# gillesdegottex/percivaltts

Hardware: AMD Instinct MI355X
Metric: acoustic frames/sec per WGAN-GP critic+gen step (higher is better)
Workload: dtype f32

## Files before the change

include/percival_hip.h:

```cpp
#ifndef PERCIVAL_HIP_H
#define PERCIVAL_HIP_H

#include <stddef.h>
#include <stdint.h>

#ifdef __cplusplus
extern "C" {
#endif

#define PTTS_OK            0
#define PTTS_EINVAL       -1
#define PTTS_ELAUNCH      -2
#define PTTS_EWORKSPACE   -3
#define PTTS_EDEVICE      -4

#define PTTS_IN_NONE     0
#define PTTS_IN_LRELU    1
#define PTTS_IN_MASKMUL  2

#define PTTS_PAD_SAME    0
#define PTTS_PAD_CAUSAL  1

#define PTTS_ACT_NONE    0
#define PTTS_ACT_LRELU   1
#define PTTS_ACT_SIGMOID 2
#define PTTS_ACT_TANH    3

const char* ptts_version(void);
const char* ptts_device_arch(void);
const char* ptts_last_error(void);
int ptts_device_status(unsigned* word_out);
int ptts_device_status_clear(void);
unsigned* ptts_device_status_word(void);
int ptts_device_status_message(unsigned word, char* buf, size_t n);
int ptts_set_deterministic(int on);
int ptts_get_deterministic(void);
int ptts_set_bf16_products(int on);
int ptts_get_bf16_products(void);

int ptts_conv2d_fwd(const float* x, const float* w, const float* bias ,
                    const float* in_scale , const float* in_shift ,
                    const float* mask_src ,
                    float* y,
                    int B, int T, int F, int Cin, int Cout, int KT, int KF,
                    int dil_t, int pad_mode, int in_mode, float alpha, void* stream);

size_t ptts_conv2d_bwd_workspace_bytes(int B, int T, int F, int Cin, int Cout, int KT, int KF, int dil_t);
int ptts_conv2d_bwd(const float* dy, const float* x, const float* w,
                    const float* in_scale, const float* in_shift, const float* mask_src,
                    float* dx, float* dw, float* dbias, float* dscale, float* dshift,
                    void* workspace, size_t workspace_bytes,
                    int B, int T, int F, int Cin, int Cout, int KT, int KF,
                    int dil_t, int pad_mode, int in_mode, float alpha, void* stream);

int ptts_conv2d_bwd_partials(const float* dy, const float* x, const float* w, const float* mask_src,
                             float* dx, void* workspace, size_t workspace_bytes, int* nblocks_out,
                             int B, int T, int F, int Cin, int Cout, int KT, int KF,
                             int dil_t, int pad_mode, int in_mode, float alpha, void* stream);
typedef struct ptts_conv2d_reduce_desc {
    const float* partials;
    int nblocks, npart, nw, cout;
    float* dw; float* dbias;
} ptts_conv2d_reduce_desc;
int ptts_conv2d_reduce_grouped(const ptts_conv2d_reduce_desc* descs, int n, void* stream);

int ptts_conv2d_mfma_supported(int F, int Cin, int Cout, int KT, int KF, int dil_t);
size_t ptts_conv2d_mfma_table_bytes(int KT);
int ptts_conv2d_mfma_tables(const float* w, void* table_fwd, void* table_bwd, int KT, int KF, int Cin, int Cout,
                            int planes , void* stream);
int ptts_conv2d_mfma_tables_grouped(const float* const* w, void* const* table_fwd, void* const* table_bwd, int n, int planes,
                                    void* stream);
int ptts_conv2d_mfma_fwd(const void* x, const void* table, const float* bias, const float* in_scale, const float* in_shift,
                         const void* mask_src, const void* out_mask, void* y,
                         int B, int T, int F, int KT, int dil_t, int pad_t, int in_mode, float alpha,
                         int planes, int in_bf16, int out_bf16, void* stream);
int ptts_conv2d_mfma_fwd_stats_supported(int F, int dil_t, int in_mode);
int ptts_conv2d_mfma_fwd_stats(const float* x, const void* table, const float* bias, const float* in_scale, const float* in_shift,
                               float* y, int B, int T, int F, int KT, int pad_t, int in_mode, float alpha,
                               double* stats, int capacity_rows, int* nrows_out, void* stream);
size_t ptts_conv2d_mfma_wgrad_workspace_bytes(int B, int T);
int ptts_conv2d_mfma_wgrad_partials(const void* dy, const void* x, const void* mask_src, void* workspace,
                                    size_t workspace_bytes, int* nblocks_out, int* npart_out, int B, int T, int F,
                                    int KT, int dil_t, int pad_t, int in_mode, float alpha,
                                    int planes, int x_bf16, int dy_bf16, void* stream);
size_t ptts_conv2d_mfma_bwd_fused_workspace_bytes(int B, int T);
int ptts_conv2d_mfma_bwd_fused_supported(int F, int dil_t, int planes);
int ptts_conv2d_mfma_bwd_fused(const void* p, const void* q, const void* mask_src, const void* table, void* y,
                               void* workspace, size_t workspace_bytes, int* nblocks_out, int* npart_out,
                               int B, int T, int F, int KT, int pad_t, int kind, float alpha, void* stream);
int ptts_conv2d_mfma_bwd_fused_affine(const float* p, const float* q, const void* table, float* y, void* workspace, size_t workspace_bytes,
                                      int* nblocks_out, int* npart_out, int B, int T, int F, int KT, int pad_t, float alpha,
                                      const float* q_scale, const float* q_shift, void* stream);
int ptts_conv2d_mfma_debug(int flags, void* stamp_buf);

int ptts_conv2d_chain_supported(int F, int L, int Cin0, int C, int KT, int KF);
int ptts_conv2d_chain_debug(void* stamp_buf);
size_t ptts_conv2d_chain_tables_bytes(void);
size_t ptts_conv2d_chain_partials_bytes(int L);
long long ptts_conv2d_chain_map_elems(int B, int T, int F);
int ptts_conv2d_chain_tables(const float* const* w, const float* const* b, void* tables, int L, int cin0, void* stream);
int ptts_conv2d_chain_fwd(const float* x0, long long ldx, const void* tables, void* maps, void* a_last,
                          int B, int T, int F, int L, float alpha, void* stream);
int ptts_conv2d_chain_bwd(const void* d_last, int d_bf16, const float* x0, long long ldx, const void* maps, const void* a_last,
                          const void* tables, float* partials, size_t partials_bytes, int* nblocks_out, int* npart_out,
                          int B, int T, int F, int L, int cin0, float alpha, void* stream);
int ptts_conv2d_chain_bwd_data(const void* d_last, int d_bf16, const void* maps, const void* a_last, const void* tables,
                               void* gmaps, float* g0, int B, int T, int F, int L, float alpha, void* stream);
int ptts_conv2d_chain_second(const float* u0, const void* gmaps, const void* maps, const void* a_last, const void* tables,
                             void* out, int out_bf16, float* partials, size_t partials_bytes, int* nblocks_out, int* npart_out,
                             int B, int T, int F, int L, int cin0, float alpha, void* stream);

int ptts_gemm(const float* A, const float* Bm, const float* bias, float* C,
              int M, int N, int K,
              int transA, long long lda, long long rows_per_seg, long long seg_stride,
              int transB, long long ldb, long long ldc,
              int in_mode, const float* in_scale, const float* in_shift, const float* mask_src,
              float alpha, int accumulate, const float* out_mask, float* colsum_b, void* stream);

typedef struct ptts_wgrad_desc {
    const float* A; const float* B; float* C; float* colsum_b;
    const float* in_scale; const float* in_shift; const float* mask_src;
    int M, N, K;
    long long lda, ldb, ldc;
    int in_mode; float alpha;
} ptts_wgrad_desc;
int ptts_gemm_wgrad_grouped(const ptts_wgrad_desc* descs, int n, void* stream);

size_t ptts_dense_planes_bytes(int N, int K);
int ptts_split3_dense_weight(const float* w, long long ldw, int K, int N, int transposed, void* planes, void* stream);
typedef struct ptts_dense_split_desc {
    const float* w; void* planes;
    long long ldw;
    int K, N, transposed, reserved;
} ptts_dense_split_desc;
int ptts_split3_dense_weight_grouped(const ptts_dense_split_desc* descs, int n, void* stream);
int ptts_split3_frame_windows(const float* x, int B, int T, int C, int NS, int S, int row_off, int P, int kvalid,
                              void* planes, long long stride_planes_bytes, void* stream);
int ptts_split3_dense_weight_strided(const float* w, long long stride_w, void* planes, long long stride_planes_bytes, int n,
                                     long long ldw, int K, int N, int transposed, void* stream);
int ptts_dense_bf16x6_supported(int M, int N, int K, long long lda, long long ldc);
typedef struct ptts_dense_wgrad_reduce_desc {
    const float* partials;
    int split, Kin, N;
    long long ldc;
    float* C; float* colsum_b;
} ptts_dense_wgrad_reduce_desc;
int ptts_dense_wgrad_bf16x6_supported(int Kin, int N, int M, long long lda, long long ldb);
size_t ptts_dense_wgrad_workspace_bytes(int Kin, int N, int M);
int ptts_dense_wgrad_bf16x6_partials(const float* A, const float* dY, const float* mask_src, const float* in_scale,
                                     const float* in_shift, void* workspace, size_t workspace_bytes, int* split_out,
                                     int Kin, int N, int M, long long lda, long long ldb, int in_mode, float alpha,
                                     void* stream);
int ptts_dense_wgrad_reduce_grouped(const ptts_dense_wgrad_reduce_desc* descs, int n, void* stream);
int ptts_dense_wgrad_bf16x6(const float* A, const float* dY, const float* mask_src, const float* in_scale,
                            const float* in_shift, float* C, float* colsum_b, void* workspace, size_t workspace_bytes,
                            int Kin, int N, int M, long long lda, long long ldb, long long ldc, int in_mode, float alpha,
                            void* stream);
int ptts_dense_bf16x6(const float* A, const void* planes, const float* bias, float* C, int M, int N, int K,
                      long long lda, long long ldc, int in_mode, const float* in_scale, const float* in_shift,
                      const float* mask_src, float alpha, int accumulate, const float* out_mask, void* stream);
int ptts_dense_bf16x6_res(const float* A, const void* planes, const float* bias, float* C, int M, int N, int K,
                          long long lda, long long ldc, int in_mode, const float* in_scale, const float* in_shift,
                          const float* mask_src, float alpha, const float* res, int res_rows, long long ldr,
                          const float* out_mask, void* stream);
int ptts_dense_bf16x6_stats_rows(int M, int N);
int ptts_dense_bf16x6_stats(const float* A, const void* planes, const float* bias, float* C, int M, int N, int K,
                            long long lda, long long ldc, int in_mode, const float* in_scale, const float* in_shift,
                            float alpha, double* stats, int capacity_rows, int* nrows_out, void* stream);
int ptts_dense_bf16x6_bwd_affine(const float* A, const void* planes, float* C, int M, int N, int K, long long lda, long long ldc,
                                 const float* z, const float* scale, const float* shift, float alpha,
                                 double* stats, int capacity_rows, int* nrows_out, void* stream);
int ptts_partial_rows_sum(const double* partials, int nrows, int ncols, double* out, void* stream);
int ptts_dft_mirror(float* Ap, int NB, int B, int Cin, int Kh, void* stream);

int ptts_conv1d_freq_kernel_planes(const float* w, const float* tw, void* planes, int NB, int KW, int Cin, int N, int Kh, void* stream);

int ptts_transpose_batched(const float* src, float* dst, int nb, int rows, int cols, void* stream);
int ptts_conv1d_freq_wgrad_combine(const float* out2, float* dW, int KW, int Cin, int N, int Kh, void* stream);

size_t ptts_conv1d_freq_wgrad_inverse_workspace_bytes(int KW, int Cin, int N);
int ptts_conv1d_freq_wgrad_inverse(const float* Gt, const float* t2, float* dW, void* workspace, size_t workspace_bytes,
                                   int NB, int NBp, int KW, int Cin, int N, int Kh, void* stream);

#define PTTS_PLANES_ROWS 0x100
typedef struct ptts_dense_rows_desc {
    const float* B;
    long long strideB, ldb;
    int windows, nB, T, NS, S, row_off;
    int kvalid, mirror_cols;
} ptts_dense_rows_desc;
int ptts_dense_bf16x6_batched(const float* A, long long strideA, const void* planes, long long stride_planes_bytes,
                              const float* bias, float* C, long long strideC, int nbatch, int M, int N, int K,
                              long long lda, long long ldc, int planes_count, void* stream);
int ptts_set_dense_batched_resident(int on);
int ptts_dense_batched_resident_enabled(void);
int ptts_dense_batched_resident_eligible(long long strideA, int M, int N, int K, int planes_count);
int ptts_dense_tn_bf16x6_batched(const float* A, long long strideA, const float* B, long long strideB, float* C, long long strideC,
                                 int nbatch, int M, int Kin, int N, long long lda, long long ldb, long long ldc, int planes_count,
                                 void* stream);

int ptts_split3_frames(const float* x, void* p1, void* p2, void* p3, int B, int T, int C, int pad_left, int pad_right,
                       int Cp, void* stream);
int ptts_split3_weight_t(const float* w, void* p1, void* p2, void* p3, int KW, int C, int N, int Cp, void* stream);
int ptts_conv1d_bf16x6(const void* a1, const void* a2, const void* a3, const void* bt1, const void* bt2, const void* bt3,
                       const float* bias, float* y, int B, int T, int KW, int Cp, int N, void* stream);

int ptts_split3_frames_t(const float* x, void* p1, void* p2, void* p3, int B, int T, int C, int pad_left, int Tp, int Crows,
                         long long Pp, void* stream);
int ptts_conv1d_wgrad_bf16x6(const void* xt1, const void* xt2, const void* xt3, const void* yt1, const void* yt2,
                             const void* yt3, float* dw, int B, int T, int KW, int C, int N, int Crows, long long Pp,
                             void* stream);

int ptts_transpose_frames(const float* x, float* out, int B, int T, int C, int pad_left, int Tp, int Crows, long long Pp,
                          void* stream);
int ptts_conv1d_wgrad_t(const float* xt, const float* yt, float* dw, float* db, int B, int T, int KW, int C, int N, int Crows,
                        long long Pp, void* stream);

size_t ptts_colstats_workspace_bytes(long long rows, int C);
int ptts_colstats(const float* x, long long rows, int C,
                  int in_mode, const float* in_scale, const float* in_shift, const float* mask_src, float alpha,
                  double* sums , void* workspace, size_t workspace_bytes, void* stream);

int ptts_bn_finalize(const double* sums, long long count, const float* gamma, const float* beta,
                     float* moving_mean, float* moving_var, float eps, float momentum,
                     int training, int update_moving, int unbiased_moving, int C,
                     float* scale, float* shift, float* mean , float* rstd , void* stream);

int ptts_bn_batch_stats_supported(long long rows, int C);
int ptts_bn_batch_stats(const float* x, long long rows, int C, const float* gamma, const float* beta,
                        float* moving_mean, float* moving_var, float eps, float momentum, int update_moving, int unbiased_moving,
                        float* scale, float* shift, float* mean , float* rstd ,
                        void* workspace, size_t workspace_bytes, int* counter, void* stream);

int ptts_bn_finalize_partials(const double* partials, int nrows, long long rows, int C, const float* gamma, const float* beta,
                              float* moving_mean, float* moving_var, float eps, float momentum, int update_moving, int unbiased_moving,
                              float* scale, float* shift, float* mean , float* rstd , void* stream);

int ptts_bn_bwd_coefs(const float* dscale, const float* dshift, const float* mean, const float* rstd,
                      const float* gamma , long long count, int C,
                      float* dgamma, float* dbeta, float* c0, float* c2, void* stream);
int ptts_bn_bwd_coefs_acc(const float* dscale, const float* dshift, const float* mean, const float* rstd,
                      const float* gamma , long long count, int C,
                      float* dgamma, float* dbeta, float* c0, float* c2, void* stream);

int ptts_affine_act(const float* x, const float* scale, const float* shift, float* y,
                    long long rows, int C, int act, float alpha, void* stream);
int ptts_affine_act_bwd(const float* dy, const float* x, const float* y, const float* scale, const float* shift,
                        float* dx, double* dsums ,
                        void* workspace, size_t workspace_bytes,
                        long long rows, int C, int act, float alpha, void* stream);
int ptts_gated_mul_fwd(const float* a, const float* b, float* y, long long n, void* stream);
int ptts_gated_mul_bwd(const float* dy, const float* a, const float* b, float* da, float* db, long long n, void* stream);

int ptts_axpby_cols(const float* a, const float* c1, const float* x, const float* c2, const float* c0,
                    float* out, long long rows, int C, void* stream);

int ptts_gp_interpolate(const float* real, const float* fake, const float* alpha_b , float* out,
                        int B, long long TD, void* stream);
int ptts_gp_sqnorm(const float* g, float* out, int B, long long TD, void* stream);
int ptts_gp_penalty(const float* sq , float* penalty , float* coef , int B, void* stream);
int ptts_gp_scale_rows(const float* g, const float* coef, const float* upstream , float* dg,
                       int B, long long TD, void* stream);

int ptts_mean_scaled(const float* v, long long n, float sign, float* out, void* stream);
int ptts_wlse_fwd(const float* y, const float* yhat, const float* w , float* out,
                  long long rows, int D, void* stream);
int ptts_wlse_bwd(const float* y, const float* yhat, const float* w, const float* upstream, float* dyhat,
                  long long rows, int D, void* stream);

int ptts_weight_clip(float* p, long long n, float lo, float hi, void* stream);

int ptts_adam_keras_step(float* p, const float* g, float* m, float* v, long long n,
                         float lr, float b1, float b2, float eps, float gscale,
                         int* step , void* stream);

size_t ptts_lstm_fwd_workspace_bytes(int B, int T, int H, int ndir);
int ptts_lstm_fwd(const float* xproj, const float* U, float* h_out, float* gates, float* c_out,
                  void* workspace, size_t workspace_bytes,
                  int B, int T, int H, int ndir, int reverse, void* stream);
size_t ptts_lstm_bwd_workspace_bytes(int B, int T, int H, int ndir);
int ptts_lstm_bwd(const float* dh_out , const float* U, const float* gates, const float* c_out,
                  float* dgates, void* workspace, size_t workspace_bytes,
                  int B, int T, int H, int ndir, int reverse, void* stream);
int ptts_lstm_graph_stats(unsigned long long* hits, unsigned long long* captures, unsigned long long* direct);

size_t ptts_gru_fwd_workspace_bytes(int B, int T, int H, int ndir);
int ptts_gru_fwd(const float* xproj, const float* U, float* h_out, float* gates, float* rh,
                 void* workspace, size_t workspace_bytes, int B, int T, int H, int ndir, void* stream);
size_t ptts_gru_bwd_workspace_bytes(int B, int T, int H, int ndir);
int ptts_gru_bwd(const float* dh_out , const float* U, const float* h_out, const float* gates,
                 float* dgates, void* workspace, size_t workspace_bytes, int B, int T, int H, int ndir, void* stream);

size_t ptts_mlpg_workspace_bytes(int B, int T, int D);
int ptts_mlpg(const float* y, const float* mean, const float* std, const float* var, int var_per_frame,
              const float* wins, const int* lengths, float* out, void* workspace, size_t workspace_bytes,
              int B, int T, int D, int K, void* stream);

#define PTTS_NORM_MEANSTD 0
#define PTTS_NORM_MINMAX  1
size_t ptts_compose_windows_workspace_bytes(int N, int D, int K);
int ptts_compose_windows(const float* y, const int* offsets, const double* wins, int mlpg_order, float* out,
                         float* run_min, float* run_max, double* run_sum, int n_stat_utts, void* workspace,
                         size_t workspace_bytes, int N, int R, int D, int K, void* stream);
size_t ptts_compose_sqdev_workspace_bytes(int N, int W);
int ptts_compose_sqdev(const float* y, const int* offsets, const double* mean, double* run_sq, int n_stat_utts,
                       void* workspace, size_t workspace_bytes, int N, int R, int W, void* stream);
int ptts_compose_normalise(const float* y, const int* keepidx, const float* a, const float* b, int mode, float scale,
                           float offset, float* out, long long R, int Win, int Wout, void* stream);

size_t ptts_mcep_table_bytes(int M1, int dftlen);
int ptts_mcep_table(float* table, size_t table_bytes, int M1, double alpha, int dftlen, void* stream);
size_t ptts_fwbnd_table_bytes(int dftlen);
int ptts_fwbnd_table(double* table, size_t table_bytes, int nb, double fs, double alpha, int dftlen, void* stream);
int ptts_mcep_postfilter(const float* mcep, float* out, int T, int M1, double alpha, int dftlen, double pf_coef,
                         const float* table, size_t table_bytes, void* stream);
int ptts_mcep2spec(const float* mcep, float* spec, int T, int M1, double alpha, int dftlen, int log_out, int postfilter,
                   double pf_coef, const float* table, size_t table_bytes, void* stream);
int ptts_fwbnd2spec(const float* fw, float* spec, int T, int nb, double fs, double alpha, int dftlen, int log_out,
                    int postfilter, double pf_coef, const double* table, size_t table_bytes, void* stream);
size_t ptts_spec2mcep_table_bytes(int M1, int dftlen);
int ptts_spec2mcep_table(double* table, size_t table_bytes, int M1, double alpha, int dftlen, void* stream);
int ptts_spec2mcep(const float* x, float* out, int T, int M1, double alpha, int dftlen, int is_log, const double* table,
                   size_t table_bytes, void* stream);

int ptts_noise_mask(const float* nmb, const float* f0, float* out, int T, int nb, double fs, int dftlen, const double* table,
                    size_t table_bytes, void* stream);
int ptts_pulse_segments(const float* spec, const float* mask, const float* noise, const int* itab, const double* dtab, int P, int T,
                        int dftlen, double fs, long long wavlen, float* seg, int W, void* stream);
int ptts_pulse_overlap_add(const float* seg, const int* itab, int P, int W, float* wav, long long wavlen, void* stream);

int ptts_aper_rows(const float* aper, const float* vuv, float* out, int T, int nb, double fs, int dftlen, const double* table,
                   size_t table_bytes, void* stream);
int ptts_world_segments(const float* spec, const float* aper, const float* noise, const int* itab, const double* dtab, int P, int T,
                        int dftlen, double fs, long long wavlen, float* seg, int W, void* stream);

#define PTTS_COMPRESS_MEAN 0
#define PTTS_COMPRESS_LSQ  1
int ptts_frame_harmonics(const float* wav, long long N, const float* f0, float* spec, float* u, int T, int Hcap, double shift,
                         double fs, int dftlen, int log_out, void* stream);
int ptts_phase_coherence(const float* u, const float* f0, float* R, float* nm, int T, int Hcap, int nb, double shift, double fs,
                         int dftlen, const double* fwtable, size_t fwtable_bytes, const double* ctable, size_t ctable_bytes,
                         void* stream);
size_t ptts_fwbnd_compress_table_bytes(int nb);
int ptts_fwbnd_compress_table(double* ctable, size_t ctable_bytes, const double* fwtable, size_t fwtable_bytes, int nb, int dftlen,
                              void* stream);
int ptts_fwbnd_compress(const float* x, float* out, int T, int nb, int dftlen, int mode, int is_log, const double* fwtable,
                        size_t fwtable_bytes, const double* ctable, size_t ctable_bytes, void* stream);

int ptts_world_envelope(const float* wav, long long N, const float* rate, float* spec, int T, double shift, double fs, int dftlen,
                        int log_out, void* stream);
int ptts_world_aperiodicity(const float* wav, long long N, const float* f0, const float* voiced, float* aper, int T, int nb,
                            double shift, double fs, int dftlen, const double* fwtable, size_t fwtable_bytes, void* stream);

int ptts_f0_candidates(const float* wav, long long N, const double* rw, size_t rw_bytes, float* freq, float* strength, int* n,
                       int* lag, float* r, int T, int ncand, double shift, double fs, int dftlen, double f0_min, double f0_max,
                       double gpeak, double voicing_threshold, double silence_threshold, double octave_cost, void* stream);
int ptts_f0_viterbi_max_frames(int ncand);
int ptts_f0_viterbi(const float* freq, const float* strength, const int* n, float* f0, int* path, int T, int ncand, double shift,
                    double octave_jump_cost, double voiced_unvoiced_cost, void* stream);
int ptts_f0_refine(const float* wav, long long N, const float* f0, float* out, int* status , int T,
                   double shift, double fs, double f0_min, double f0_max, void* stream);

int ptts_resample(const float* x, const long long* x_off, long long total_in, float* y, const long long* y_off,
                  long long total_out, long long max_out, int n_utts, const double* h, size_t h_bytes, int up, int down, int hw,
                  void* stream);
int ptts_highpass_tile(int* chunk, int* tile);
int ptts_highpass_sections(double fs, double fc, double* sos);
// ... 41 lines not shown
```

percivaltts_amd/csrc/common.h:

```cpp
#pragma once
#include <hip/hip_runtime.h>
#include <cstdio>
#include <cstdarg>
#include "../../include/percival_hip.h"

namespace ptts {

void set_error(const char* fmt, ...);
bool deterministic();
bool bf16_products();
int zero_f32(float* p, size_t n, hipStream_t st);
int zero_f32_2d(float* p, size_t ld, size_t cols, size_t rows, hipStream_t st);

constexpr int STATUS_SLOT_C2M = 0, STATUS_SLOT_LSTM = 1, STATUS_SLOTS = 2;
constexpr unsigned STATUS_C2M_HANDOFF = 0x1u;
constexpr unsigned STATUS_LSTM_HANDOFF = 0x2u;
unsigned* status_words();
int check_status(const char* what);
__device__ __forceinline__ void raise_status(unsigned* words, int slot, unsigned code) {
    __hip_atomic_store(words + slot, code, __ATOMIC_RELAXED, __HIP_MEMORY_SCOPE_SYSTEM);
}

inline int check_launch(const char* what) {
    hipError_t e = hipGetLastError();
    if (e != hipSuccess) {
        set_error("%s: launch failed: %s", what, hipGetErrorString(e));
        return PTTS_ELAUNCH;
    }
    return PTTS_OK;
}

#define PTTS_REQUIRE(cond, ...)                         \
    do {                                                \
        if (!(cond)) {                                  \
            ptts::set_error(__VA_ARGS__);               \
            return PTTS_EINVAL;                         \
        }                                               \
    } while (0)

constexpr int WAVE = 64;

int thin_gemm_dispatch(const float* A, const float* Bm, const float* bias, float* C, int M, int N, int K, int transA,
                       long long lda, long long rows_per_seg, long long seg_stride, int transB, long long ldb,
                       long long ldc, int in_mode, const float* in_scale, const float* in_shift,
                       const float* mask_src, float alpha, int accumulate, const float* out_mask, hipStream_t st);

__device__ __forceinline__ float lrelu(float p, float alpha) { return p > 0.f ? p : alpha * p; }
__device__ __forceinline__ float lrelu_d(float p, float alpha) { return p > 0.f ? 1.f : alpha; }

__device__ __forceinline__ float wave_sum(float v) {
#pragma unroll
    for (int o = 32; o > 0; o >>= 1) v += __shfl_xor(v, o, 64);
    return v;
}
__device__ __forceinline__ double wave_sum(double v) {
#pragma unroll
    for (int o = 32; o > 0; o >>= 1) v += __shfl_xor(v, o, 64);
    return v;
}

inline size_t align_up(size_t v, size_t a) { return (v + a - 1) / a * a; }

}
```

percivaltts_amd/csrc/conv2d.hip:

```cpp
#include "common.h"
#include <cstdlib>

namespace ptts {

template <int C> struct VecIO;
template <> struct VecIO<1> {
    static __device__ __forceinline__ void ld(const float* p, float* v) { v[0] = p[0]; }
    static __device__ __forceinline__ void st(float* p, const float* v) { p[0] = v[0]; }
};
template <> struct VecIO<2> {
    static __device__ __forceinline__ void ld(const float* p, float* v) {
        float2 t = *reinterpret_cast<const float2*>(p); v[0] = t.x; v[1] = t.y; }
    static __device__ __forceinline__ void st(float* p, const float* v) {
        *reinterpret_cast<float2*>(p) = make_float2(v[0], v[1]); }
};
template <> struct VecIO<4> {
    static __device__ __forceinline__ void ld(const float* p, float* v) {
        float4 t = *reinterpret_cast<const float4*>(p); v[0] = t.x; v[1] = t.y; v[2] = t.z; v[3] = t.w; }
    static __device__ __forceinline__ void st(float* p, const float* v) {
        *reinterpret_cast<float4*>(p) = make_float4(v[0], v[1], v[2], v[3]); }
};

constexpr int CONV_THREADS = 256;

// ... 648 lines not shown
}

__global__ void conv2d_bwd_dx_generic(const float* __restrict__ dy, const float* __restrict__ x,
                                      const float* __restrict__ w, const float* __restrict__ in_scale,
                                      const float* __restrict__ in_shift, float* __restrict__ dx,
                                      long long total, int T, int F, int Cin, int Cout, int KT, int KF,
                                      int dil_t, int pad_t, int in_mode, float alpha) {
    const int PF = (KF - 1) / 2;
    for (long long i = blockIdx.x * (long long)blockDim.x + threadIdx.x; i < total;
         i += (long long)gridDim.x * blockDim.x) {
        const int ci = (int)(i % Cin);
        long long pix = i / Cin;
        const int f = (int)(pix % F);
        pix /= F;
        const int t = (int)(pix % T);
        const long long b = pix / T;
        float da = 0.f;
        for (int kt = 0; kt < KT; ++kt) {
            const int tt = t - kt * dil_t + pad_t;
            if (tt < 0 || tt >= T) continue;
            for (int kf = 0; kf < KF; ++kf) {
                const int ff = f - kf + PF;
                if (ff < 0 || ff >= F) continue;
                const long long base = ((b * T + tt) * F + ff) * Cout;
                for (int co = 0; co < Cout; ++co)
                    da = fmaf(dy[base + co], w[((kt * KF + kf) * Cin + ci) * Cout + co], da);
            }
        }
        if (in_mode == PTTS_IN_LRELU) {
            float p = x[i];
            if (in_scale) p = p * in_scale[ci] + in_shift[ci];
            da *= lrelu_d(p, alpha);
            if (in_scale) da *= in_scale[ci];
        }
        dx[i] = da;
    }
}

__global__ __launch_bounds__(256) void conv2d_bwd_w_generic(
    const float* __restrict__ dy, const float* __restrict__ x, const float* __restrict__ w,
    const float* __restrict__ in_scale, const float* __restrict__ in_shift,
    const float* __restrict__ mask_src, float* __restrict__ dw, float* __restrict__ dbias,
    float* __restrict__ dscale, float* __restrict__ dshift, long long npix, int T, int F, int Cin,
    int Cout, int KT, int KF, int dil_t, int pad_t, int in_mode, float alpha) {
    __shared__ double sh[4];
    const int PF = (KF - 1) / 2;
    const int NW = KT * KF * Cin * Cout;
    const int j = blockIdx.x;
    double s = 0.0;
    if (j < NW) {
        const int co = j % Cout, ci = (j / Cout) % Cin, kf = (j / (Cout * Cin)) % KF, kt = j / (Cout * Cin * KF);
        for (long long pix = threadIdx.x; pix < npix; pix += 256) {
            const int f = (int)(pix % F);
            const int t = (int)((pix / F) % T);
            const long long b = pix / ((long long)F * T);
            const int tt = t + kt * dil_t - pad_t, ff = f + kf - PF;
            if (tt < 0 || tt >= T || ff < 0 || ff >= F) continue;
            const long long off = ((b * T + tt) * F + ff) * Cin + ci;
            s += (double)(gen_in(x, in_scale, in_shift, mask_src, off, ci, in_mode, alpha) * dy[pix * Cout + co]);
        }
    } else if (j < NW + Cout) {
        const int co = j - NW;
        for (long long pix = threadIdx.x; pix < npix; pix += 256) s += (double)dy[pix * Cout + co];
    } else {
        const int which = (j - NW - Cout) / Cin, ci = (j - NW - Cout) % Cin;
        for (long long pix = threadIdx.x; pix < npix; pix += 256) {
            const int f = (int)(pix % F);
            const int t = (int)((pix / F) % T);
            const long long b = pix / ((long long)F * T);
            float da = 0.f;
            for (int kt = 0; kt < KT; ++kt) {
                const int tt = t - kt * dil_t + pad_t;
                if (tt < 0 || tt >= T) continue;
                for (int kf = 0; kf < KF; ++kf) {
                    const int ff = f - kf + PF;
                    if (ff < 0 || ff >= F) continue;
                    const long long base = ((b * T + tt) * F + ff) * Cout;
                    for (int co = 0; co < Cout; ++co)
                        da = fmaf(dy[base + co], w[((kt * KF + kf) * Cin + ci) * Cout + co], da);
                }
            }
            const float xr = x[pix * Cin + ci];
            const float p = xr * in_scale[ci] + in_shift[ci];
            da *= lrelu_d(p, alpha);
            s += (double)(which == 0 ? da * xr : da);
        }
    }
    s = wave_sum(s);
    if ((threadIdx.x & 63) == 0) sh[threadIdx.x >> 6] = s;
    __syncthreads();
    if (threadIdx.x == 0) {
        const float v = (float)(sh[0] + sh[1] + sh[2] + sh[3]);
        if (j < NW) { if (dw) dw[j] = v; }
        else if (j < NW + Cout) { if (dbias) dbias[j - NW] = v; }
        else if (j < NW + Cout + Cin) { if (dscale) dscale[j - NW - Cout] = v; }
        else { if (dshift) dshift[j - NW - Cout - Cin] = v; }
    }
}

static bool conv_use_mfma() {
    static int v = -1;
    if (v < 0) { const char* e = getenv("PTTS_CONV_MFMA"); v = e ? atoi(e) : 0; }
    return v != 0;
}

static size_t lds_budget() {
    static size_t v = 0;
    if (!v) {
        const char* e = getenv("PTTS_CONV_LDS_KB");
        v = (size_t)(e ? atoi(e) : 48) * 1024;
        if (v < 8 * 1024) v = 8 * 1024;
        if (v > 150 * 1024) v = 150 * 1024;
    }
    return v;
}

struct Tile { int TT; int ntiles; };

static Tile pick_tile(int T, int F, int KT, int KF, int dil_t, size_t bytes_per_row_fixed,
                      size_t bytes_per_halo_row) {
    const int nspr = (F + KF - 1) / KF;
    const int halo = (KT - 1) * dil_t;
    Tile best{0, 0};
    double best_score = -1.0;
    for (int TT = 4; TT <= 128; ++TT) {
        const size_t lds = (size_t)TT * bytes_per_row_fixed + (size_t)(TT + halo) * bytes_per_halo_row;
        if (lds > lds_budget() && best.TT > 0) break;
        const int ntiles = (T + TT - 1) / TT;
        const int strips = TT * nspr;
        const int rounds = (strips + CONV_THREADS - 1) / CONV_THREADS;
        const double lane_eff = (double)strips / (rounds * CONV_THREADS);
        const double row_eff = (double)T / ((double)ntiles * TT);
        const double halo_eff = (double)TT / (TT + halo);
        const double score = lane_eff * row_eff * (0.75 + 0.25 * halo_eff);
        if (score > best_score + 1e-9) { best_score = score; best = Tile{TT, ntiles}; }
    }
    return best;
}

static Tile pick_tile_fwd(int T, int F, int KT, int KF, int dil_t, int cols) {
    const int nspr = (F + KF - 1) / KF;
    const int halo = (KT - 1) * dil_t;
    if (const char* e = getenv("PTTS_CONV_TT")) {
        const int TT = atoi(e);
        if (TT > 0 && (TT + halo) * cols <= NPF * CONV_THREADS) return Tile{TT, (T + TT - 1) / TT};
    }
    Tile best{0, 0};
    double best_score = -1.0;
    for (int TT = 1; TT <= 128; ++TT) {
        if ((TT + halo) * cols > NPF * CONV_THREADS) break;
        const int strips = TT * nspr;
        const int rounds = (strips + CONV_THREADS - 1) / CONV_THREADS;
        if (rounds > 2) break;
        const int ntiles = (T + TT - 1) / TT;
        const double lane_eff = (double)strips / (rounds * CONV_THREADS);
        const double row_eff = (double)T / ((double)ntiles * TT);
        const double halo_eff = (double)TT / (TT + halo);
        const double score = lane_eff * row_eff * (0.6 + 0.4 * halo_eff);
        if (score > best_score + 1e-9) { best_score = score; best = Tile{TT, ntiles}; }
    }
    return best;
}

struct ConvGeom {
    int pad_t;
    bool ok;
};
static ConvGeom geom(int KT, int dil_t, int pad_mode) {
    ConvGeom g;
    const int span = (KT - 1) * dil_t;
    g.pad_t = pad_mode == PTTS_PAD_CAUSAL ? span : span / 2;
    g.ok = true;
    return g;
}

#define PTTS_CONV_CASES(M)                                                                    \
    M(1, 1, 3, 3) M(1, 2, 3, 3) M(1, 4, 3, 3) M(2, 1, 3, 3) M(2, 2, 3, 3) M(2, 4, 3, 3)       \
    M(4, 1, 3, 3) M(4, 2, 3, 3) M(4, 4, 3, 3)                                                 \
    M(1, 1, 5, 5) M(1, 2, 5, 5) M(1, 4, 5, 5) M(2, 1, 5, 5) M(2, 2, 5, 5) M(2, 4, 5, 5)       \
    M(4, 1, 5, 5) M(4, 2, 5, 5) M(4, 4, 5, 5)

}

using namespace ptts;

extern "C" int ptts_conv2d_fwd(const float* x, const float* w, const float* bias, const float* in_scale,
                               const float* in_shift, const float* mask_src, float* y, int B, int T, int F,
                               int Cin, int Cout, int KT, int KF, int dil_t, int pad_mode, int in_mode,
                               float alpha, void* stream) {
    PTTS_REQUIRE(x && w && y, "conv2d_fwd: null tensor");
    PTTS_REQUIRE(B > 0 && T > 0 && F > 0 && Cin > 0 && Cout > 0 && KT > 0 && KF > 0 && dil_t > 0,
                 "conv2d_fwd: bad dims B=%d T=%d F=%d Cin=%d Cout=%d KT=%d KF=%d dil=%d", B, T, F, Cin, Cout, KT, KF, dil_t);
    PTTS_REQUIRE(in_mode >= 0 && in_mode <= 2, "conv2d_fwd: bad in_mode %d", in_mode);
    PTTS_REQUIRE((in_scale == nullptr) == (in_shift == nullptr), "conv2d_fwd: scale/shift must come together");
    PTTS_REQUIRE(in_mode != PTTS_IN_MASKMUL || mask_src, "conv2d_fwd: MASKMUL needs mask_src");
    PTTS_REQUIRE(B <= 65535, "conv2d_fwd: B too large");
    hipStream_t st = (hipStream_t)stream;
    const ConvGeom g = geom(KT, dil_t, pad_mode);
#define FWD_LAUNCH(CI, CO, KTT, KFF, NRR, MK)                                                           \
    hipLaunchKernelGGL((conv2d_fwd_kernel<CI, CO, KTT, KFF, NRR, MK>), dim3(grid), dim3(CONV_THREADS), lds, \
                       st, x, w, bias, in_scale, in_shift, mask_src, y, T, F, tl.TT, tl.ntiles,             \
                       tl.ntiles * B, dil_t, g.pad_t, in_mode, alpha)
#define FWD_CASE(CI, CO, KTT, KFF)                                                                       \
    if (Cin == CI && Cout == CO && KT == KTT && KF == KFF) {                                             \
        const int nspr = (F + KFF - 1) / KFF;                                                            \
        const int cols = nspr * KFF + KFF - 1;                                                           \
        const Tile tl = pick_tile_fwd(T, F, KTT, KFF, dil_t, cols);                                      \
        const int rows = tl.TT + (KTT - 1) * dil_t;                                                      \
        const size_t in_fl = ((size_t)rows * cols * CI + 3) & ~(size_t)3;                                \
        const size_t lds = (in_fl + (size_t)tl.TT * F * CO) * sizeof(float);                             \
        const int nr = (tl.TT * nspr + CONV_THREADS - 1) / CONV_THREADS;                                 \
        if (tl.TT > 0 && lds <= 150 * 1024 && nr <= 2 && rows * cols <= NPF * CONV_THREADS) {            \
            int per_cu = (int)((150 * 1024) / lds);                                                      \
            if (per_cu > 4) per_cu = 4;                                                                  \
            long long grid = (long long)tl.ntiles * B;                                                   \
            if (grid > 256LL * per_cu) grid = 256LL * per_cu;                                            \
            const bool mk = in_mode == PTTS_IN_MASKMUL;                                                  \
            if (conv_use_mfma() && dil_t >= 1) {                                                         \
                if (mk) hipLaunchKernelGGL((conv2d_fwd_mfma_kernel<CI, CO, KTT, KFF, true, 2>), dim3(grid), dim3(CONV_THREADS), lds, st, x, w, bias, in_scale, in_shift, mask_src, y, T, F, tl.TT, tl.ntiles, tl.ntiles * B, dil_t, g.pad_t, in_mode, alpha); \
                else hipLaunchKernelGGL((conv2d_fwd_mfma_kernel<CI, CO, KTT, KFF, false, 2>), dim3(grid), dim3(CONV_THREADS), lds, st, x, w, bias, in_scale, in_shift, mask_src, y, T, F, tl.TT, tl.ntiles, tl.ntiles * B, dil_t, g.pad_t, in_mode, alpha); \
                return check_launch("conv2d_fwd_mfma");                                                  \
            }                                                                                            \
            if (nr == 1) { if (mk) FWD_LAUNCH(CI, CO, KTT, KFF, 1, true); else FWD_LAUNCH(CI, CO, KTT, KFF, 1, false); } \
            else { if (mk) FWD_LAUNCH(CI, CO, KTT, KFF, 2, true); else FWD_LAUNCH(CI, CO, KTT, KFF, 2, false); }         \
            return check_launch("conv2d_fwd");                                                           \
        }                                                                                                \
    }
    PTTS_CONV_CASES(FWD_CASE)
#undef FWD_CASE
#undef FWD_LAUNCH
    const long long total = (long long)B * T * F * Cout;
    const int blocks = (int)((total + 255) / 256 < 65536 ? (total + 255) / 256 : 65536);
    hipLaunchKernelGGL(conv2d_fwd_generic, dim3(blocks), dim3(256), 0, st, x, w, bias, in_scale, in_shift,
                       mask_src, y, total, T, F, Cin, Cout, KT, KF, dil_t, g.pad_t, in_mode, alpha);
    return check_launch("conv2d_fwd_generic");
}

namespace {
constexpr size_t WT_BYTES = 4096;
struct BwdPlan { bool fast; Tile tl; size_t lds; int npart; };
template <int CI, int CO, int KTT, int KFF>
BwdPlan plan_bwd(int T, int F, int dil_t) {
    BwdPlan p;
    const int nspr = (F + KFF - 1) / KFF;
    const int Fp = nspr * KFF;
    const size_t halo_row = (size_t)(Fp + KFF - 1) * CO * sizeof(float);
    const size_t fixed_row = (size_t)Fp * CI * sizeof(float) * 2;
    p.tl = pick_tile(T, F, KTT, KFF, dil_t, fixed_row, halo_row);
    p.lds = (size_t)p.tl.TT * fixed_row + (size_t)(p.tl.TT + (KTT - 1) * dil_t) * halo_row;
    constexpr int NW = KTT * KFF * CI * CO;
    constexpr int NGRP = CONV_THREADS / (KTT * CI);
    const size_t red = ((size_t)NGRP * NW + 4 * (CO + 2 * CI)) * sizeof(float);
    if (p.lds < red) p.lds = red;
    p.npart = NW + CO + 2 * CI;
    p.fast = p.lds <= 160 * 1024 - 256;
    return p;
}
}

extern "C" size_t ptts_conv2d_bwd_workspace_bytes(int B, int T, int F, int Cin, int Cout, int KT, int KF,
                                                  int dil_t) {
#define WS_CASE(CI, CO, KTT, KFF)                                                      \
    if (Cin == CI && Cout == CO && KT == KTT && KF == KFF) {                           \
        const BwdPlan p = plan_bwd<CI, CO, KTT, KFF>(T, F, dil_t);                     \
        if (p.fast) return WT_BYTES + (size_t)B * p.tl.ntiles * p.npart * sizeof(float); \
    }
    PTTS_CONV_CASES(WS_CASE)
#undef WS_CASE
    return 16;
}

static int conv2d_bwd_impl(const float* dy, const float* x, const float* w, const float* in_scale,
                           const float* in_shift, const float* mask_src, float* dx, float* dw,
                           float* dbias, float* dscale, float* dshift, void* workspace,
                           size_t workspace_bytes, int B, int T, int F, int Cin, int Cout, int KT, int KF,
                           int dil_t, int pad_mode, int in_mode, float alpha, void* stream, int partials_only,
                           int* nblocks_out) {
    PTTS_REQUIRE(dy && x && w, "conv2d_bwd: null tensor");
    PTTS_REQUIRE(B > 0 && T > 0 && F > 0 && Cin > 0 && Cout > 0 && KT > 0 && KF > 0 && dil_t > 0,
                 "conv2d_bwd: bad dims");
    PTTS_REQUIRE(in_mode >= 0 && in_mode <= 2, "conv2d_bwd: bad in_mode %d", in_mode);
    PTTS_REQUIRE((in_scale == nullptr) == (in_shift == nullptr), "conv2d_bwd: scale/shift must come together");
    PTTS_REQUIRE(in_mode != PTTS_IN_MASKMUL || mask_src, "conv2d_bwd: MASKMUL needs mask_src");
    PTTS_REQUIRE(!(in_mode == PTTS_IN_MASKMUL && dx), "conv2d_bwd: dx is not defined for MASKMUL (weight-only sweep)");
    PTTS_REQUIRE((dscale == nullptr) == (dshift == nullptr), "conv2d_bwd: dscale/dshift must come together");
    PTTS_REQUIRE(!dscale || (in_mode == PTTS_IN_LRELU && in_scale), "conv2d_bwd: dscale needs LRELU with scale/shift");
    PTTS_REQUIRE(B <= 65535, "conv2d_bwd: B too large");
    hipStream_t st = (hipStream_t)stream;
    const ConvGeom g = geom(KT, dil_t, pad_mode);
    const int want_dx = dx != nullptr, want_dw = (dw != nullptr || dbias != nullptr || partials_only), want_aff = dscale != nullptr;
    if (!want_dx && !want_dw && !want_aff) return PTTS_OK;
#define BWD_CASE(CI, CO, KTT, KFF)                                                                         \
    if (Cin == CI && Cout == CO && KT == KTT && KF == KFF) {                                               \
        const BwdPlan p = plan_bwd<CI, CO, KTT, KFF>(T, F, dil_t);                                         \
        if (p.fast) {                                                                                      \
            const int nblocks = B * p.tl.ntiles;                                                           \
            const size_t need = WT_BYTES + (size_t)nblocks * p.npart * sizeof(float);                      \
            if (!workspace || workspace_bytes < need) {                                                    \
                set_error("conv2d_bwd: workspace %zu < %zu", workspace_bytes, need);                       \
                return PTTS_EWORKSPACE;                                                                    \
            }                                                                                              \
            float* wt = (float*)workspace;                                                                 \
            float* parts = (float*)((char*)workspace + WT_BYTES);                                          \
            hipLaunchKernelGGL((conv2d_bwd_kernel<CI, CO, KTT, KFF>), dim3(p.tl.ntiles, B),                \
                               dim3(CONV_THREADS), p.lds, st, dy, x, w, in_scale, in_shift, mask_src, dx,  \
                               parts, (const float*)wt, want_dx, want_dw, want_aff, T, F, p.tl.TT, dil_t,  \
                               g.pad_t, in_mode, alpha);                                                   \
            int rc = check_launch("conv2d_bwd");                                                           \
            if (rc) return rc;                                                                             \
            if (nblocks_out) *nblocks_out = nblocks;                                                       \
            if ((want_dw || want_aff) && !partials_only) {                                                 \
                hipLaunchKernelGGL(reduce_partials_kernel, dim3(p.npart), dim3(256), 0, st,                \
                                   (const float*)parts, nblocks, p.npart, want_dw ? dw : nullptr,          \
                                   KTT * KFF * CI * CO, want_dw ? dbias : nullptr, CO, dscale, dshift, CI);\
                rc = check_launch("conv2d_bwd_reduce");                                                    \
            }                                                                                              \
            return rc;                                                                                     \
        }                                                                                                  \
    }
    PTTS_CONV_CASES(BWD_CASE)
#undef BWD_CASE
    PTTS_REQUIRE(!partials_only, "conv2d_bwd_partials: this shape has no tiled kernel (workspace_bytes == 16): use ptts_conv2d_bwd");
    const long long npix = (long long)B * T * F;
    if (want_dx) {
        const long long total = npix * Cin;
        const int blocks = (int)((total + 255) / 256 < 65536 ? (total + 255) / 256 : 65536);
        hipLaunchKernelGGL(conv2d_bwd_dx_generic, dim3(blocks), dim3(256), 0, st, dy, x, w, in_scale, in_shift,
                           dx, total, T, F, Cin, Cout, KT, KF, dil_t, g.pad_t, in_mode, alpha);
        int rc = check_launch("conv2d_bwd_dx_generic");
        if (rc) return rc;
    }
    if (want_dw || want_aff) {
        const int nw = KT * KF * Cin * Cout;
        const int nblk = nw + Cout + (want_aff ? 2 * Cin : 0);
        hipLaunchKernelGGL(conv2d_bwd_w_generic, dim3(nblk), dim3(256), 0, st, dy, x, w, in_scale, in_shift,
                           mask_src, want_dw ? dw : nullptr, want_dw ? dbias : nullptr, dscale, dshift, npix, T,
                           F, Cin, Cout, KT, KF, dil_t, g.pad_t, in_mode, alpha);
        return check_launch("conv2d_bwd_w_generic");
    }
    return PTTS_OK;
}

extern "C" int ptts_conv2d_bwd(const float* dy, const float* x, const float* w, const float* in_scale,
                               const float* in_shift, const float* mask_src, float* dx, float* dw,
                               float* dbias, float* dscale, float* dshift, void* workspace,
                               size_t workspace_bytes, int B, int T, int F, int Cin, int Cout, int KT, int KF,
                               int dil_t, int pad_mode, int in_mode, float alpha, void* stream) {
    return conv2d_bwd_impl(dy, x, w, in_scale, in_shift, mask_src, dx, dw, dbias, dscale, dshift, workspace, workspace_bytes,
                           B, T, F, Cin, Cout, KT, KF, dil_t, pad_mode, in_mode, alpha, stream, 0, nullptr);
}

extern "C" int ptts_conv2d_bwd_partials(const float* dy, const float* x, const float* w, const float* mask_src,
                                        float* dx, void* workspace, size_t workspace_bytes, int* nblocks_out,
                                        int B, int T, int F, int Cin, int Cout, int KT, int KF,
                                        int dil_t, int pad_mode, int in_mode, float alpha, void* stream) {
    PTTS_REQUIRE(nblocks_out, "conv2d_bwd_partials: nblocks_out is NULL");
    return conv2d_bwd_impl(dy, x, w, nullptr, nullptr, mask_src, dx, nullptr, nullptr, nullptr, nullptr, workspace,
                           workspace_bytes, B, T, F, Cin, Cout, KT, KF, dil_t, pad_mode, in_mode, alpha, stream, 1, nblocks_out);
}

constexpr int RG_MAX = 16;
struct ReduceGroupArgs {
    int n;
    int col_begin[RG_MAX + 1];
    const float* partials[RG_MAX]; int nblocks[RG_MAX], npart[RG_MAX], nw[RG_MAX], ncout[RG_MAX];
    float* dw[RG_MAX]; float* dbias[RG_MAX];
};

constexpr int RG_COLS = 64, RG_ROWS = 4, RG_SLAB = 128;
__global__ __launch_bounds__(RG_COLS * RG_ROWS) void conv2d_reduce_grouped_kernel(ReduceGroupArgs a) {
    __shared__ double sh[RG_ROWS][RG_COLS];
    int gi = 0;
    while ((int)blockIdx.x >= a.col_begin[gi + 1]) ++gi;
    const int cx = threadIdx.x & (RG_COLS - 1), ry = threadIdx.x / RG_COLS;
    const int npart = a.npart[gi], nblocks = a.nblocks[gi], ncols = a.nw[gi] + a.ncout[gi];
    const int nchunks = (ncols + RG_COLS - 1) / RG_COLS, r = blockIdx.x - a.col_begin[gi];
    const int slab = r / nchunks, j = (r - slab * nchunks) * RG_COLS + cx;
    const int row_end = min(nblocks, (slab + 1) * RG_SLAB);
    const float* p = a.partials[gi] + j;
    double s0 = 0.0, s1 = 0.0, s2 = 0.0, s3 = 0.0;
    if (j < ncols) {
        int blk = slab * RG_SLAB + ry;
        for (; blk + 3 * RG_ROWS < row_end; blk += 4 * RG_ROWS) {
            const float v0 = p[(size_t)blk * npart], v1 = p[(size_t)(blk + RG_ROWS) * npart];
            const float v2 = p[(size_t)(blk + 2 * RG_ROWS) * npart], v3 = p[(size_t)(blk + 3 * RG_ROWS) * npart];
            s0 += (double)v0; s1 += (double)v1; s2 += (double)v2; s3 += (double)v3;
        }
        for (; blk < row_end; blk += RG_ROWS) s0 += (double)p[(size_t)blk * npart];
    }
    sh[ry][cx] = (s0 + s1) + (s2 + s3);
    __syncthreads();
    if (ry == 0 && j < ncols) {
        double t = sh[0][cx];
#pragma unroll
        for (int q = 1; q < RG_ROWS; ++q) t += sh[q][cx];
        const float v = (float)t;
        if (j < a.nw[gi]) { if (a.dw[gi]) atomicAdd(a.dw[gi] + j, v); }
        else if (a.dbias[gi]) atomicAdd(a.dbias[gi] + (j - a.nw[gi]), v);
    }
}

extern "C" int ptts_conv2d_reduce_grouped(const ptts_conv2d_reduce_desc* descs, int n, void* stream) {
    PTTS_REQUIRE(descs && n > 0, "conv2d_reduce_grouped: nothing to reduce");
    for (int base = 0; base < n; base += RG_MAX) {
        ReduceGroupArgs a;
        a.n = n - base < RG_MAX ? n - base : RG_MAX;
        int cols = 0;
        for (int i = 0; i < a.n; ++i) {
            const ptts_conv2d_reduce_desc& d = descs[base + i];
            PTTS_REQUIRE(d.partials && d.nblocks > 0 && d.nw > 0 && d.cout > 0 && d.npart >= d.nw + d.cout,
                         "conv2d_reduce_grouped: bad pass %d", base + i);
            a.col_begin[i] = cols;
            cols += ((d.nw + d.cout + RG_COLS - 1) / RG_COLS) * ((d.nblocks + RG_SLAB - 1) / RG_SLAB);
            a.partials[i] = d.partials; a.nblocks[i] = d.nblocks; a.npart[i] = d.npart; a.nw[i] = d.nw; a.ncout[i] = d.cout;
            a.dw[i] = d.dw; a.dbias[i] = d.dbias;
        }
        a.col_begin[a.n] = cols;
        hipLaunchKernelGGL(conv2d_reduce_grouped_kernel, dim3(cols), dim3(RG_COLS * RG_ROWS), 0, (hipStream_t)stream, a);
        int rc = check_launch("conv2d_reduce_grouped");
        if (rc) return rc;
    }
    return PTTS_OK;
}
```

Measured before the change: 4.858 million.

## Add specialized persistent backward kernel for 5x5 single-input-channel edge conv

```diff
diff --git a/include/percival_hip.h b/include/percival_hip.h
--- a/include/percival_hip.h
+++ b/include/percival_hip.h
@@ -63,6 +63,9 @@
     float* dw; float* dbias;
 } ptts_conv2d_reduce_desc;
 int ptts_conv2d_reduce_grouped(const ptts_conv2d_reduce_desc* descs, int n, void* stream);
+
+int ptts_set_conv2d_edge(int on);
+int ptts_conv2d_edge_eligible(int Cin, int Cout, int KT, int KF, int dil_t, int in_mode, int F);
 
 int ptts_conv2d_mfma_supported(int F, int Cin, int Cout, int KT, int KF, int dil_t);
 size_t ptts_conv2d_mfma_table_bytes(int KT);
diff --git a/percivaltts_amd/csrc/common.h b/percivaltts_amd/csrc/common.h
--- a/percivaltts_amd/csrc/common.h
+++ b/percivaltts_amd/csrc/common.h
@@ -45,6 +45,10 @@
                        long long ldc, int in_mode, const float* in_scale, const float* in_shift,
                        const float* mask_src, float alpha, int accumulate, const float* out_mask, hipStream_t st);
 
+int conv2d_edge_bwd(const float* dy, const float* x, const float* w, const float* in_scale, float* dx, float* partials,
+                    int want_dx, int want_dw, int want_affine, int max_rows, int* nrows_out, int B, int T, int F, int Cin,
+                    int Cout, int KT, int KF, int dil_t, int pad_t, int in_mode, hipStream_t st);
+
 __device__ __forceinline__ float lrelu(float p, float alpha) { return p > 0.f ? p : alpha * p; }
 __device__ __forceinline__ float lrelu_d(float p, float alpha) { return p > 0.f ? 1.f : alpha; }
 
diff --git a/percivaltts_amd/csrc/conv2d.hip b/percivaltts_amd/csrc/conv2d.hip
--- a/percivaltts_amd/csrc/conv2d.hip
+++ b/percivaltts_amd/csrc/conv2d.hip
@@ -974,16 +974,21 @@
             }                                                                                              \
             float* wt = (float*)workspace;                                                                 \
             float* parts = (float*)((char*)workspace + WT_BYTES);                                          \
-            hipLaunchKernelGGL((conv2d_bwd_kernel<CI, CO, KTT, KFF>), dim3(p.tl.ntiles, B),                \
-                               dim3(CONV_THREADS), p.lds, st, dy, x, w, in_scale, in_shift, mask_src, dx,  \
-                               parts, (const float*)wt, want_dx, want_dw, want_aff, T, F, p.tl.TT, dil_t,  \
-                               g.pad_t, in_mode, alpha);                                                   \
+            int nrows = nblocks;    \
+            const int edge = conv2d_edge_bwd(dy, x, w, in_scale, dx, parts, want_dx, want_dw, want_aff, nblocks, &nrows, \
+                                             B, T, F, Cin, Cout, KT, KF, dil_t, g.pad_t, in_mode, st);     \
+            if (edge < 0) return PTTS_ELAUNCH;                                                             \
+            if (edge == 0)                                                                                 \
+                hipLaunchKernelGGL((conv2d_bwd_kernel<CI, CO, KTT, KFF>), dim3(p.tl.ntiles, B),            \
+                                   dim3(CONV_THREADS), p.lds, st, dy, x, w, in_scale, in_shift, mask_src, dx, \
+                                   parts, (const float*)wt, want_dx, want_dw, want_aff, T, F, p.tl.TT, dil_t, \
+                                   g.pad_t, in_mode, alpha);                                               \
             int rc = check_launch("conv2d_bwd");                                                           \
             if (rc) return rc;                                                                             \
-            if (nblocks_out) *nblocks_out = nblocks;                                                       \
+            if (nblocks_out) *nblocks_out = nrows;                                                         \
             if ((want_dw || want_aff) && !partials_only) {                                                 \
                 hipLaunchKernelGGL(reduce_partials_kernel, dim3(p.npart), dim3(256), 0, st,                \
-                                   (const float*)parts, nblocks, p.npart, want_dw ? dw : nullptr,          \
+                                   (const float*)parts, nrows, p.npart, want_dw ? dw : nullptr,            \
                                    KTT * KFF * CI * CO, want_dw ? dbias : nullptr, CO, dscale, dshift, CI);\
                 rc = check_launch("conv2d_bwd_reduce");                                                    \
             }                                                                                              \
diff --git a/percivaltts_amd/csrc/conv2d_edge.hip b/percivaltts_amd/csrc/conv2d_edge.hip
--- /dev/null
+++ b/percivaltts_amd/csrc/conv2d_edge.hip
@@ -0,0 +1,282 @@
+#include "common.h"
+#include <cstdint>
+#include <cstdlib>
+
+namespace ptts {
+namespace c2e {
+
+constexpr int THREADS = 256;
+constexpr int K = 5;
+constexpr int HALO = K - 1;
+constexpr int CO = 4;
+constexpr int NW = K * K * CO;
+constexpr int NSUM = NW + CO;
+constexpr int NPART = NW + CO + 2;
+constexpr int NPD = 7;
+constexpr int MAX_GRID = 512;
+constexpr int RCH = 26, RSTRIDE = RCH + 1, RPARTS = 8;
+constexpr size_t RED_BYTES = ((size_t)THREADS * RSTRIDE + RPARTS * RCH) * sizeof(float);
+static_assert(NSUM % RCH == 0, "whole chunks");
+
+typedef float f2 __attribute__((ext_vector_type(2)));
+__device__ __forceinline__ f2 pkfma(float a, f2 w, f2 c) { return __builtin_elementwise_fma((f2){a, a}, w, c); }
+
+template <bool DX, bool DW>
+struct Regs {
+    float4 dyh[DX ? NPD : 1];
+    float xh[DW ? NPD : 1];
+    float4 g[(DW && !DX) ? K : 1];
+};
+
+template <bool DX, bool DW>
+__device__ __forceinline__ void prefetch(Regs<DX, DW>& pf, const float* __restrict__ dy, const float* __restrict__ x,
+                                         long long img, int t0, int T, int F, int pad_t, const int* rel, const int* rrow,
+                                         bool has_strip, int r, int fs) {
+    if (DX) {
+        const int t_org = t0 - (HALO - pad_t);
+#pragma unroll
+        for (int u = 0; u < NPD; ++u) {
+            pf.dyh[u] = make_float4(0.f, 0.f, 0.f, 0.f);
+            const int t = t_org + rrow[u];
+            if (t >= 0 && t < T)
+                pf.dyh[u] = *reinterpret_cast<const float4*>(dy + (img + (long long)t_org * F + rel[u]) * CO);
+        }
+    }
+    if (DW) {
+        const int t_org = t0 - pad_t;
+#pragma unroll
+        for (int u = 0; u < NPD; ++u) {
+            pf.xh[u] = 0.f;
+            const int t = t_org + rrow[u];
+            if (t >= 0 && t < T) pf.xh[u] = x[img + (long long)t_org * F + rel[u]];
+        }
+    }
+    if (DW && !DX) {
+        const int t = t0 + r;
+#pragma unroll
+        for (int p = 0; p < K; ++p) {
+            pf.g[p] = make_float4(0.f, 0.f, 0.f, 0.f);
+            if (has_strip && t < T && fs + p < F)
+                pf.g[p] = *reinterpret_cast<const float4*>(dy + (img + (long long)t * F + fs + p) * CO);
+        }
+    }
+}
+
+template <bool DX, bool DW>
+__global__ __launch_bounds__(THREADS) void bwd_kernel(const float* __restrict__ dy, const float* __restrict__ x,
+                                                      const float* __restrict__ w, float* __restrict__ dx,
+                                                      float* __restrict__ partials, int T, int F, int TT, int ntiles_t,
+                                                      int nitems, int pad_t) {
+    extern __shared__ __attribute__((aligned(16))) float smem[];
+    const int nspr = (F + K - 1) / K;
+    const int cols = nspr * K + HALO;
+    const int total = (TT + HALO) * cols;
+    float4* dyt = reinterpret_cast<float4*>(smem);
+    float* xt = smem + (DX ? (size_t)total * CO : 0);
+    const int tid = threadIdx.x;
+    const int lo_t = HALO - pad_t;
+
+    const bool has_strip = tid < TT * nspr;
+    const int r = has_strip ? tid / nspr : 0;
+    const int fs = has_strip ? (tid - r * nspr) * K : 0;
+
+    int rel[NPD], rrow[NPD];
+#pragma unroll
+    for (int u = 0; u < NPD; ++u) {
+        const int idx = tid + u * THREADS;
+        const int rr = idx / cols, f = idx - rr * cols - 2;
+        const bool ok = idx < total && f >= 0 && f < F;
+        rel[u] = ok ? rr * F + f : 0;
+        rrow[u] = ok ? rr : -(1 << 28);
+    }
+
+    f2 acc[K][K][2];
+    float sb[CO];
+    if (DW) {
+#pragma unroll
+        for (int kt = 0; kt < K; ++kt)
+#pragma unroll
+            for (int kf = 0; kf < K; ++kf) { acc[kt][kf][0] = (f2){0.f, 0.f}; acc[kt][kf][1] = (f2){0.f, 0.f}; }
+#pragma unroll
+        for (int co = 0; co < CO; ++co) sb[co] = 0.f;
+    }
+
+    Regs<DX, DW> pf;
+    int item = blockIdx.x;
+    if (item < nitems) {
+        const int b = item / ntiles_t, t0 = (item - b * ntiles_t) * TT;
+        prefetch<DX, DW>(pf, dy, x, (long long)b * T * F, t0, T, F, pad_t, rel, rrow, has_strip, r, fs);
+    }
+    while (item < nitems) {
+        const int b = item / ntiles_t, t0 = (item - b * ntiles_t) * TT;
+        const long long img = (long long)b * T * F;
+#pragma unroll
+        for (int u = 0; u < NPD; ++u) {
+            const int idx = tid + u * THREADS;
+            if (idx < total) {
+                if (DX) dyt[idx] = pf.dyh[u];
+                if (DW) xt[idx] = pf.xh[u];
+            }
+        }
+        float4 g[K];
+        if (DW && !DX) {
+#pragma unroll
+            for (int p = 0; p < K; ++p) g[p] = pf.g[p];
+        }
+        __syncthreads();
+        const int next = item + gridDim.x;
+        if (next < nitems) {
+            const int nb = next / ntiles_t, nt0 = (next - nb * ntiles_t) * TT;
+            prefetch<DX, DW>(pf, dy, x, (long long)nb * T * F, nt0, T, F, pad_t, rel, rrow, has_strip, r, fs);
+        }
+        const bool act = has_strip && t0 + r < T;
+
+        if (DX && act) {
+            f2 da2[K];
+#pragma unroll
+            for (int p = 0; p < K; ++p) da2[p] = (f2){0.f, 0.f};
+#pragma unroll 1
+            for (int kt = 0; kt < K; ++kt) {
+                const float4* row = dyt + (size_t)(r + (K - 1 - kt)) * cols + fs;
+#pragma unroll
+                for (int j = 0; j < 2 * K - 1; ++j) {
+                    const float4 gv = row[j];
+#pragma unroll
+                    for (int kf = 0; kf < K; ++kf) {
+                        const int p = j - (K - 1 - kf);
+                        if (p < 0 || p >= K) continue;
+                        const f2* wk2 = reinterpret_cast<const f2*>(w + (kt * K + kf) * CO);
+                        da2[p] = __builtin_elementwise_fma((f2){gv.x, gv.y}, wk2[0], da2[p]);
+                        da2[p] = __builtin_elementwise_fma((f2){gv.z, gv.w}, wk2[1], da2[p]);
+                    }
+                }
+            }
+            float* dxo = dx + img + (long long)(t0 + r) * F + fs;
+#pragma unroll
+            for (int p = 0; p < K; ++p)
+                if (fs + p < F) dxo[p] = da2[p].x + da2[p].y;
+        }
+
+        if (DW && act) {
+            if (DX) {
+#pragma unroll
+                for (int p = 0; p < K; ++p) g[p] = dyt[(size_t)(r + lo_t) * cols + fs + p + 2];
+            }
+#pragma unroll
+            for (int p = 0; p < K; ++p) { sb[0] += g[p].x; sb[1] += g[p].y; sb[2] += g[p].z; sb[3] += g[p].w; }
+#pragma unroll
+            for (int kt = 0; kt < K; ++kt) {
+                const float* xrow = xt + (size_t)(r + kt) * cols + fs;
+                float xv[2 * K - 1];
+#pragma unroll
+                for (int j = 0; j < 2 * K - 1; ++j) xv[j] = xrow[j];
+#pragma unroll
+                for (int p = 0; p < K; ++p)
+#pragma unroll
+                    for (int kf = 0; kf < K; ++kf) {
+                        acc[kt][kf][0] = pkfma(xv[p + kf], (f2){g[p].x, g[p].y}, acc[kt][kf][0]);
+                        acc[kt][kf][1] = pkfma(xv[p + kf], (f2){g[p].z, g[p].w}, acc[kt][kf][1]);
+                    }
+            }
+        }
+        __syncthreads();
+        item = next;
+    }
+
+    if (DW) {
+        float* red = smem;
+        float* red2 = smem + (size_t)THREADS * RSTRIDE;
+        float* out = partials + (size_t)blockIdx.x * NPART;
+#pragma unroll
+        for (int ch = 0; ch < NSUM / RCH; ++ch) {
+#pragma unroll
+            for (int i = 0; i < RCH; ++i) {
+                const int s = ch * RCH + i;
+                float v;
+                if (s < NW) {
+                    const f2 a = acc[s / (K * CO)][(s / CO) % K][(s % CO) / 2];
+                    v = (s % 2) ? a.y : a.x;
+                } else {
+                    v = sb[s - NW];
+                }
+                red[tid * RSTRIDE + i] = v;
+            }
+            __syncthreads();
+            if (tid < RPARTS * RCH) {
+                const int part = tid / RCH, i = tid - part * RCH;
+                float s = 0.f;
+#pragma unroll 8
+                for (int l = 0; l < THREADS / RPARTS; ++l) s += red[(part * (THREADS / RPARTS) + l) * RSTRIDE + i];
+                red2[part * RCH + i] = s;
+            }
+            __syncthreads();
+            if (tid < RCH) {
+                float s = 0.f;
+#pragma unroll
+                for (int part = 0; part < RPARTS; ++part) s += red2[part * RCH + tid];
+                out[ch * RCH + tid] = s;
+            }
+        }
+        if (tid < NPART - NSUM) out[NSUM + tid] = 0.f;
+    }
+}
+
+static int g_edge = -1;
+static int edge_on() {
+    if (g_edge < 0) { const char* e = getenv("PTTS_CONV2D_EDGE"); g_edge = e ? (atoi(e) != 0 ? 1 : 0) : 1; }
+    return g_edge;
+}
+
+static int tile_rows(int T, int F) {
+    const int nspr = (F + K - 1) / K;
+    const int cols = nspr * K + HALO;
+    int TT = THREADS / nspr;
+    const int by_regs = NPD * THREADS / cols - HALO;
+    if (by_regs < TT) TT = by_regs;
+    if (T < TT) TT = T;
+    return TT < 1 ? 0 : TT;
+}
+
+}
+
+int conv2d_edge_bwd(const float* dy, const float* x, const float* w, const float* in_scale, float* dx, float* partials,
+                    int want_dx, int want_dw, int want_affine, int max_rows, int* nrows_out, int B, int T, int F, int Cin,
+                    int Cout, int KT, int KF, int dil_t, int pad_t, int in_mode, hipStream_t st) {
+    using namespace c2e;
+    if (!edge_on() || !ptts_conv2d_edge_eligible(Cin, Cout, KT, KF, dil_t, in_mode, F)) return 0;
+    if (in_scale || want_affine || ((uintptr_t)dy & 15) != 0 || max_rows < 1) return 0;
+    const int TT = tile_rows(T, F);
+    const int ntiles_t = (T + TT - 1) / TT;
+    const long long nitems = (long long)B * ntiles_t;
+    long long grid = nitems < MAX_GRID ? nitems : MAX_GRID;
+    if (grid > max_rows) grid = max_rows;
+    const int nspr = (F + K - 1) / K;
+    const size_t total = (size_t)(TT + HALO) * (nspr * K + HALO);
+    size_t lds = total * sizeof(float) * ((want_dx ? CO : 0) + (want_dw ? 1 : 0));
+    if (want_dw && lds < RED_BYTES) lds = RED_BYTES;
+#define C2E_LAUNCH(DXV, DWV)                                                                                            \
+    hipLaunchKernelGGL((bwd_kernel<DXV, DWV>), dim3((unsigned)grid), dim3(THREADS), lds, st, dy, x, w, dx, partials, T, \
+                       F, TT, ntiles_t, (int)nitems, pad_t)
+    if (want_dx && want_dw) C2E_LAUNCH(true, true);
+    else if (want_dx) C2E_LAUNCH(true, false);
+    else C2E_LAUNCH(false, true);
+#undef C2E_LAUNCH
+    const int rc = check_launch("conv2d_edge_bwd");
+    if (rc) return -1;
+    if (nrows_out) *nrows_out = (int)grid;
+    return 1;
+}
+
+}
+
+extern "C" int ptts_set_conv2d_edge(int on) {
+    const int prev = ptts::c2e::edge_on();
+    ptts::c2e::g_edge = on ? 1 : 0;
+    return prev;
+}
+
+extern "C" int ptts_conv2d_edge_eligible(int Cin, int Cout, int KT, int KF, int dil_t, int in_mode, int F) {
+    using namespace ptts::c2e;
+    return (Cin == 1 && Cout == CO && KT == K && KF == K && dil_t == 1 && in_mode == PTTS_IN_NONE && F > 0 &&
+            tile_rows(1 << 20, F) > 0) ? 1 : 0;
+}
```

After: 4.888 million (median of 5 runs). About the same (+0.6%).
